# alibaba/pairec

Measured on AMD Instinct MI355X. Metric: ranked items/sec, 5k-cand DNN rank (recall top-5000 of 100M x 128 -> DNN3 -> fuse -> sort), higher is better.
Workload: dtype bf16x3; 1 GPU; configs[1]+[2]: recall 5k of 100000000x128 fp32 table in HBM -> 3-layer DNN rank (256-512-256-1, bf16 MFMA with split hi + lo operands = bf16x3, fp32-accurate scores) -> RankScore fusion (fp64) -> ItemRankScore sort; candidates_per_request=5000, table_rows=100000000, dim=128, table_dist=uniform, batches_in_flight=2, contexts=2, all_batches_on_predicted_thresholds=True, batches_re_run_after_a_failed_plan=0, parallelism=1 GPU

## Files before the change

### pairec_amd/csrc/recall.hip

```cpp
#include "common.hpp"
#include "bitonic_reg.hpp"
#include "split_sort.hpp"

#include <type_traits>

namespace pg {

typedef float f32x16 __attribute__((ext_vector_type(16)));
typedef float f32x4 __attribute__((ext_vector_type(4)));

constexpr int kPieceRows = 32;
constexpr int kPieceCols = 32;
constexpr int kPieceBytes = kPieceRows * kPieceCols * 4;
constexpr int kPieceDmas = kPieceBytes / 1024;
constexpr int kPieceQuads = kPieceCols / 4;
constexpr int kRingSlots = 4;
constexpr int kScanWaves = 8;
constexpr int kScanLdsRing = kScanWaves * kRingSlots * kPieceBytes;
constexpr int kStageCap = 280;
constexpr int kStageBytes = kStageCap * 12 + 512;
constexpr int kScanLds = kScanLdsRing + kScanWaves * kStageBytes;

__device__ __forceinline__ uint32_t f32_ordered_bits(float f) {
    const uint32_t b = __float_as_uint(f);
// ... 683 lines not shown
                for (int r = 0; r < 16; ++r) m = fmaxf(m, __fmaf_rn((float)acc[c][r], eu[c], -nxr[r]));
                cmask[c] = __builtin_amdgcn_ballot_w64(!(m < la[c]));
            } else if constexpr (I8) {
                int m = acc[c][0];
#pragma unroll
                for (int r = 1; r < 16; ++r) m = acc[c][r] > m ? acc[c][r] : m;
                cmask[c] = __builtin_amdgcn_ballot_w64(m >= cut[c]);
            } else {
                float m = acc[c][0];
#pragma unroll
                for (int r = 1; r < 16; ++r) m = fmaxf(m, acc[c][r]);
                cmask[c] = __builtin_amdgcn_ballot_w64(!(m < cut[c]));
            }
            any_mask |= cmask[c];
        }
        if (any_mask != 0) {
            const uint32_t row0 = cur_phys * kPieceRows;
#pragma unroll
            for (int c = 0; c < NQB; ++c) {
                if (cmask[c] == 0) continue;
                uint32_t m16 = 0;
#pragma unroll
                for (int r = 0; r < 16; ++r) {
                    if constexpr (L2 == 2) {
                        const float g = __fmaf_rn((float)acc[c][r], eu[c], -nxr[r]);
                        asm volatile("v_cmp_nlt_f32 vcc, %1, %2\n\tv_addc_co_u32 %0, vcc, %0, %0, vcc"
                                     : "+v"(m16) : "v"(g), "v"(la[c]) : "vcc");
                    } else if constexpr (I8)
                        asm volatile("v_cmp_ge_i32 vcc, %1, %2\n\tv_addc_co_u32 %0, vcc, %0, %0, vcc"
                                     : "+v"(m16) : "v"(acc[c][r]), "v"(cut[c]) : "vcc");
                    else
                        asm volatile("v_cmp_nlt_f32 vcc, %1, %2\n\tv_addc_co_u32 %0, vcc, %0, %0, vcc"
                                     : "+v"(m16) : "v"(acc[c][r]), "v"(cut[c]) : "vcc");
                }
                if (row0 + kPieceRows > a.row_end) {
#pragma unroll
                    for (int r = 0; r < 16; ++r)
                        if (row0 + (r & 3) + 8 * (r >> 2) + 4 * h >= a.row_end) m16 &= ~(1u << (15 - r));
                }
                for (;;) {
                    const bool p = m16 != 0;
                    const uint64_t bm = __builtin_amdgcn_ballot_w64(p);
                    if (bm == 0) break;
                    const uint32_t n = __popcll(bm);
                    if (st_n + n > (uint32_t)kCap) flush();
                    if (p) {
                        const int r = 15 - __builtin_ctz(m16);
                        const uint32_t pos = st_n + __builtin_amdgcn_mbcnt_hi((uint32_t)(bm >> 32),
                                                 __builtin_amdgcn_mbcnt_lo((uint32_t)bm, 0u));
                        st_row[pos] = row0 + (r & 3) + 8 * (r >> 2) + 4 * h;
                        st_q[pos] = (uint32_t)(c * 32 + i32);
                        m16 &= m16 - 1;
                    }
                    st_n += n;
                }
            }
        }
    }
    }
    if constexpr (QH == 1) flush();
    wait_vmcnt<0>();
}

__device__ __forceinline__ uint32_t rec_mask(const char* r, const float* __restrict__ thr_screen, uint32_t row_end, uint32_t& q,
                                             uint32_t& row0h) {
    typedef int i32x4 __attribute__((ext_vector_type(4)));
    const uint2 tag = *reinterpret_cast<const uint2*>(r + 64);
    q = tag.y & 255u;
    const uint32_t h = (tag.y >> 8) & 1u;
    row0h = tag.x + 4 * h;
    const int t = __float_as_int(thr_screen[q]);
    uint32_t m = 0;
#pragma unroll
    for (int jj = 0; jj < 4; ++jj) {
        const i32x4 v = *reinterpret_cast<const i32x4*>(r + 16 * jj);
#pragma unroll
        for (int e = 0; e < 4; ++e) {
            const int rr = 4 * jj + e;
            if (v[e] >= t && row0h + (rr & 3) + 8 * (rr >> 2) < row_end) m |= 1u << rr;
        }
    }
    return m;
}
constexpr uint32_t kRecPoolSlice = 8192;
__global__ __launch_bounds__(1024) void screen_decode_kernel(const char* __restrict__ rec, const uint32_t* __restrict__ rec_cnt,
                                                             uint32_t rec_cap, uint32_t rec_waves, const char* __restrict__ rec_pool,
                                                             uint32_t rec_pool_cap, const float* __restrict__ thr_screen, uint32_t row_end,
                                                             uint32_t* __restrict__ susp_cnt, uint32_t* __restrict__ susp,
                                                             uint32_t cap, uint32_t* __restrict__ overflow) {
    __shared__ uint32_t cntq[kMaxQueries], baseq[kMaxQueries], nreg[8];
    constexpr uint32_t kKeep = 12288;
    __shared__ uint2 keep[kKeep];
    const bool pool = blockIdx.x >= rec_waves / 8;
    if (threadIdx.x < kMaxQueries) cntq[threadIdx.x] = 0;
    if (threadIdx.x < 8) {
        uint32_t n;
        if (pool) {
            const uint32_t filled = rec_cnt[rec_waves] < rec_pool_cap ? rec_cnt[rec_waves] : rec_pool_cap;
            const uint32_t begin = (blockIdx.x - rec_waves / 8) * kRecPoolSlice;
            n = threadIdx.x == 0 && begin < filled ? (filled - begin < kRecPoolSlice ? filled - begin : kRecPoolSlice) : 0u;
        } else {
            const uint32_t n_raw = rec_cnt[blockIdx.x * 8 + threadIdx.x];
            n = n_raw < rec_cap ? n_raw : rec_cap;
        }
        nreg[threadIdx.x] = n;
    }
    __syncthreads();
    for (int pass = 0; pass < 2; ++pass) {
        uint32_t off = 0;
        for (uint32_t w = 0; w < 8; ++w) {
            const uint32_t n = nreg[w];
            const char* const base = pool ? rec_pool + (size_t)(blockIdx.x - rec_waves / 8) * kRecPoolSlice * kRecBytes
                                          : rec + (size_t)(blockIdx.x * 8 + w) * rec_cap * kRecBytes;
            for (uint32_t e = threadIdx.x; e < n; e += 1024) {
                uint32_t q, row0h, m;
                const uint32_t slot = off + e;
                if (pass == 1 && slot < kKeep) {
                    const uint2 kp = keep[slot];
                    row0h = kp.x;
                    q = kp.y & 0xffffu;
                    m = kp.y >> 16;
                } else {
                    m = rec_mask(base + (size_t)e * kRecBytes, thr_screen, row_end, q, row0h);
                    if (pass == 0 && slot < kKeep) keep[slot] = make_uint2(row0h, q | (m << 16));
                }
                if (m == 0) continue;
                const uint32_t nh = __popc(m);
                if (pass == 0) {
                    atomicAdd(&cntq[q], nh);
                } else {
                    uint32_t pos = baseq[q] + atomicAdd(&cntq[q], nh);
                    if (pos + nh > cap) { *overflow = 1u; continue; }
                    while (m) {
                        const uint32_t rr = __builtin_ctz(m);
                        m &= m - 1;
                        susp[(uint64_t)q * cap + pos++] = row0h + (rr & 3) + 8 * (rr >> 2);
                    }
                }
            }
            off += n;
        }
        __syncthreads();
        if (pass == 0 && threadIdx.x < kMaxQueries) {
            const uint32_t c = cntq[threadIdx.x];
            baseq[threadIdx.x] = c ? atomicAdd(&susp_cnt[threadIdx.x], c) : 0u;
            cntq[threadIdx.x] = 0;
        }
        __syncthreads();
    }
}

template <int DIM>
__device__ __forceinline__ void rescore_gather(f32x4 (&buf)[16], const float* __restrict__ tab, uint32_t row, int ph, int lane) {
#pragma unroll
    for (int i = 0; i < 16; ++i) {
        const uint32_t r_i = (uint32_t)__shfl((int)row, 4 * i + (lane >> 4), 64);
        buf[i] = reinterpret_cast<const f32x4*>(tab + (size_t)r_i * DIM + ph * 64)[lane & 15];
    }
}
template <int ROWB>
__device__ __forceinline__ void rescore_walk(const f32x4 (&buf)[16], char* my, const float* qs, int ph, int lane, float& s) {
#pragma unroll
    for (int i = 0; i < 16; ++i)
        *reinterpret_cast<f32x4*>(my + (4 * i + (lane >> 4)) * ROWB + (lane & 15) * 16) = buf[i];
    __builtin_amdgcn_fence(__ATOMIC_RELEASE, "wavefront");
    __builtin_amdgcn_wave_barrier();
#pragma unroll
    for (int k = 0; k < 16; ++k) {
        const float4 x = *reinterpret_cast<const float4*>(my + lane * ROWB + k * 16);
        const float4 y = *reinterpret_cast<const float4*>(&qs[ph * 64 + 4 * k]);
        s = __fmaf_rn(x.x, y.x, s);
        s = __fmaf_rn(x.y, y.y, s);
        s = __fmaf_rn(x.z, y.z, s);
        s = __fmaf_rn(x.w, y.w, s);
        if ((k & 3) == 3) __builtin_amdgcn_sched_barrier(0);
    }
    __builtin_amdgcn_wave_barrier();
}

template <int DIM, bool L2 = false>
__global__ __launch_bounds__(256) void rescore_kernel(const float* __restrict__ tab, const float* __restrict__ qpad,
                                                      const float* __restrict__ thr,
                                                      const uint32_t* __restrict__ susp,
                                                      const uint32_t* __restrict__ susp_cnt, uint32_t cap,
                                                      uint32_t* __restrict__ cnt, uint64_t* __restrict__ cand,
                                                      uint32_t* __restrict__ overflow, uint32_t scap, uint32_t n_rows,
                                                      const float* __restrict__ nx = nullptr, const float* __restrict__ nqv = nullptr,
                                                      RowFilter filter = RowFilter()) {
    constexpr int kRowB = 64 * 4 + 16;
    __shared__ __attribute__((aligned(16))) char tile[4][64 * kRowB];
    __shared__ __attribute__((aligned(16))) float qs[DIM];
    __shared__ uint32_t wsum[4];
    __shared__ uint32_t base_s;
    const uint32_t q = blockIdx.y;
    const uint32_t n_raw = susp_cnt[q];
    const uint32_t n = n_raw < scap ? n_raw : scap;
    if (blockIdx.x * 256u >= n) return;
    const int lane = threadIdx.x & 63, w = threadIdx.x >> 6;
    if (threadIdx.x < DIM) qs[threadIdx.x] = qpad[(size_t)q * DIM + threadIdx.x];
    const float thr_q = thr[q];
    __syncthreads();
    char* const my = tile[w];
    auto row_of = [&](uint32_t t0) -> uint32_t {
        const uint32_t e = t0 + threadIdx.x;
        const uint32_t r = e < n ? susp[(uint64_t)q * scap + e] : 0u;
        return r < n_rows ? r : 0u;
    };
    constexpr int NPH = DIM / 64;
    const uint32_t step = gridDim.x * 256u;
    uint32_t t0 = blockIdx.x * 256u;
    uint32_t row = row_of(t0);
    f32x4 va[16], vb[16];
    rescore_gather<DIM>(va, tab, row, 0, lane);
    for (; t0 < n; t0 += step) {
        const bool valid = t0 + threadIdx.x < n;
        const uint32_t row_next = t0 + step < n ? row_of(t0 + step) : 0u;
        float s = 0.0f;
        if constexpr (NPH == 1) {
            rescore_gather<DIM>(vb, tab, row_next, 0, lane);
            rescore_walk<kRowB>(va, my, qs, 0, lane, s);
        } else if constexpr (NPH == 2) {
            rescore_gather<DIM>(vb, tab, row, 1, lane);
            rescore_walk<kRowB>(va, my, qs, 0, lane, s);
            rescore_gather<DIM>(va, tab, row_next, 0, lane);
            rescore_walk<kRowB>(vb, my, qs, 1, lane, s);
        } else if constexpr (NPH == 3) {
            rescore_gather<DIM>(vb, tab, row, 1, lane);
            rescore_walk<kRowB>(va, my, qs, 0, lane, s);
            rescore_gather<DIM>(va, tab, row, 2, lane);
            rescore_walk<kRowB>(vb, my, qs, 1, lane, s);
            rescore_gather<DIM>(vb, tab, row_next, 0, lane);
            rescore_walk<kRowB>(va, my, qs, 2, lane, s);
        } else {
            static_assert(NPH == 4, "rescore_kernel: DIM 64, 128, 192 or 256");
            rescore_gather<DIM>(vb, tab, row, 1, lane);
            rescore_walk<kRowB>(va, my, qs, 0, lane, s);
            rescore_gather<DIM>(va, tab, row, 2, lane);
            rescore_walk<kRowB>(vb, my, qs, 1, lane, s);
            rescore_gather<DIM>(vb, tab, row, 3, lane);
            rescore_walk<kRowB>(va, my, qs, 2, lane, s);
            rescore_gather<DIM>(va, tab, row_next, 0, lane);
            rescore_walk<kRowB>(vb, my, qs, 3, lane, s);
        }
        if (NPH & 1) {
#pragma unroll
            for (int i = 0; i < 16; ++i) va[i] = vb[i];
        }
        if constexpr (L2) s = __fmaf_rn(2.0f, s, -(nx[row] + nqv[q]));
        const bool keep = valid && !(s < thr_q) && row_filter_pass(filter, row);
        const uint64_t m = __builtin_amdgcn_ballot_w64(keep);
        const uint32_t before = __builtin_amdgcn_mbcnt_hi((uint32_t)(m >> 32), __builtin_amdgcn_mbcnt_lo((uint32_t)m, 0u));
        if (lane == 0) wsum[w] = __popcll(m);
        __syncthreads();
        if (threadIdx.x == 0) {
            const uint32_t tot = wsum[0] + wsum[1] + wsum[2] + wsum[3];
            base_s = tot ? atomicAdd(&cnt[q], tot) : 0u;
        }
        __syncthreads();
        uint32_t pos = base_s + before;
        for (int j = 0; j < w; ++j) pos += wsum[j];
        if (keep) {
            if (pos < cap) cand[(uint64_t)q * cap + pos] = topk_key(s, row);
            else *overflow = 1u;
        }
        __syncthreads();
        row = row_next;
    }
    if (n_raw > scap && threadIdx.x == 0) *overflow = 1u;
}

__global__ void screen_prep_kernel(const float* __restrict__ qpad, uint32_t dim,
                                   uint4* __restrict__ qb16, float* __restrict__ eps) {
    const uint32_t KS = dim / 16;
    const uint32_t i = blockIdx.x * blockDim.x + threadIdx.x;
    if (i < (uint32_t)kScreenMaxNQB * KS * 64) {
        const uint32_t lane = i & 63, ks = (i >> 6) % KS, c = (i >> 6) / KS;
        const float* q = qpad + (size_t)(c * 32 + (lane & 31)) * dim + ks * 16 + 8 * (lane >> 5);
        uint32_t w[4];
        for (int e = 0; e < 4; ++e) {
            auto rne = [](float x) -> uint32_t {
                uint32_t b = __float_as_uint(x);
                if ((b & 0x7FFFFFFFu) > 0x7F800000u) return (b >> 16) | 0x40u;
                b += 0x7FFFu + ((b >> 16) & 1u);
                return b >> 16;
            };
            w[e] = rne(q[2 * e]) | (rne(q[2 * e + 1]) << 16);
        }
        qb16[i] = make_uint4(w[0], w[1], w[2], w[3]);
    }
    if (i < (uint32_t)kMaxQueries) {
        double ss = 0.0;
        for (uint32_t k = 0; k < dim; ++k) {
            const double v = (double)qpad[(size_t)i * dim + k];
            ss += v * v;
        }
        eps[i] = (float)(sqrt(ss) * (double)kScreenEps * 1.0001) + 1e-30f;
    }
}

__global__ void screen_thr_kernel(const float* __restrict__ thr, const float* __restrict__ eps, float max_norm,
                                  float* __restrict__ thr_screen) {
    const uint32_t q = threadIdx.x;
    if (q >= (uint32_t)kMaxQueries) return;
    const float t = thr[q], e = eps[q];
    float v = t;
    if (!(e == e) || e > 1e28f || !(t == t) || !(e * max_norm < 1e35f)) v = -__builtin_inff();
    thr_screen[q] = v;
}

__global__ __launch_bounds__(128) void screen_prep8_kernel(const float* __restrict__ qpad, uint32_t dim,
                                                            float max_norm, float resid, uint4* __restrict__ qb8,
                                                            float* __restrict__ eps, float* __restrict__ qscale) {
    __shared__ float sq[32];
    const uint32_t tid = threadIdx.x, c = blockIdx.x;
    {
        const uint32_t ql = tid >> 2, qi = c * 32 + ql, part = tid & 3, per = dim / 4;
        const float* q = qpad + (size_t)qi * dim + part * per;
        float mx = 0.0f;
        bool bad = false;
        for (uint32_t k = 0; k < per; ++k) {
            const float v = fabsf(q[k]);
            if (!(v <= 3.0e38f)) bad = true;
            mx = fmaxf(mx, v);
        }
        mx = fmaxf(mx, __shfl_xor(mx, 1, 64));
        mx = fmaxf(mx, __shfl_xor(mx, 2, 64));
        bad = (__shfl_xor((int)bad, 1, 64) | (int)bad) != 0;
        bad = (__shfl_xor((int)bad, 2, 64) | (int)bad) != 0;
        const float sc = fmaxf(mx / 127.0f, 1e-30f);
        double ss = 0.0, dd = 0.0;
        for (uint32_t k = 0; k < per; ++k) {
            const double v = (double)q[k];
            int Q = __float2int_rn(q[k] / sc);
            Q = Q > 127 ? 127 : (Q < -127 ? -127 : Q);
            const double d = v - (double)sc * (double)Q;
            ss += v * v;
            dd += d * d;
        }
        ss += __shfl_xor(ss, 1, 64);
        ss += __shfl_xor(ss, 2, 64);
        dd += __shfl_xor(dd, 1, 64);
        dd += __shfl_xor(dd, 2, 64);
        if (part == 0) {
            const double nq = sqrt(ss), dq = sqrt(dd);
            const double e = ((double)resid * nq + ((double)max_norm + (double)resid) * dq) * 1.0001 +
                             1e-5 * (double)max_norm * nq + 1e-30;
            eps[qi] = bad ? __builtin_nanf("") : (float)(e * 1.000001);
            qscale[qi] = sc;
            sq[ql] = sc;
        }
    }
    __syncthreads();
    const uint32_t KS = dim / 32;
    for (uint32_t i = tid; i < KS * 64; i += blockDim.x) {
        const uint32_t lane = i & 63, ks = i >> 6;
        const uint32_t ql = lane & 31;
        const float* q = qpad + (size_t)(c * 32 + ql) * dim + ks * 32 + 16 * (lane >> 5);
        const float sc = sq[ql];
        uint32_t w[4];
        for (int e = 0; e < 4; ++e) {
            uint32_t word = 0;
            for (int b = 0; b < 4; ++b) {
                int Q = __float2int_rn(q[4 * e + b] / sc);
                Q = Q > 127 ? 127 : (Q < -127 ? -127 : Q);
                word |= (uint32_t)(Q & 0xff) << (8 * b);
            }
            w[e] = word;
        }
        qb8[(c * KS + ks) * 64 + lane] = make_uint4(w[0], w[1], w[2], w[3]);
    }
}

__global__ void screen_thr8_kernel(const float* __restrict__ thr, const float* __restrict__ eps,
                                   const float* __restrict__ qscale, float s_x, float* __restrict__ thr_screen) {
    const uint32_t q = threadIdx.x;
    if (q >= (uint32_t)kMaxQueries) return;
    const float t = thr[q], e = eps[q];
    int T = (int)0x80000000;
    if (e == e && e <= 1e30f && t == t && t > -__builtin_inff()) {
        const double v = floor(((double)t - (double)e) / ((double)s_x * (double)qscale[q])) - 1.0;
        T = v >= 2147483647.0 ? 0x7fffffff : (v <= -2147483648.0 ? (int)0x80000000 : (int)v);
    }
    thr_screen[q] = __int_as_float(T);
}

__global__ void screen_thr8_l2_kernel(const float* __restrict__ thr, const float* __restrict__ eps, const float* __restrict__ qscale,
                                      const float* __restrict__ nqv, float s_x, float max_norm, float* __restrict__ a_out,
                                      float* __restrict__ b_out, int per_row) {
    const uint32_t q = threadIdx.x;
    if (q >= (uint32_t)kMaxQueries) return;
    const float t = thr[q], e = eps[q];
    const double nq = (double)nqv[q], N = (double)max_norm;
    const double sq = (double)s_x * (double)qscale[q];
    float A = -__builtin_inff(), B = 0.0f;
    if (e == e && e <= 1e30f && t == t && t > -__builtin_inff() && sq > 0.0 && nq == nq && nq < 1e30) {
        const double delta = 2e-6 * (N * N + nq + 2.0 * N * sqrt(nq)) + 1e-30;
        if (per_row) {
            const double c = (double)t - 2.0 * delta + nq - 2.0 * (double)e;
            A = (float)(c - fabs(c) * 1e-6 - 1e-30);
            B = (float)(2.0 * sq);
            if (!(A == A) || !(B == B) || B > 1e30f) { A = -__builtin_inff(); B = 0.0f; }
        } else {
            const double a = (((double)t - delta + nq) * 0.5 - (double)e) / sq;
            const double b = 0.5 / sq;
            A = (float)(a - fabs(a) * 1e-6 - 1.0);
            B = (float)(b * (1.0 - 1e-6));
            if (!(A == A) || !(B == B) || B > 1e30f) { A = -__builtin_inff(); B = 0.0f; }
        }
    }
    a_out[q] = A;
    b_out[q] = B;
}
__global__ void block_nxmin_kernel(const float* __restrict__ nx, uint64_t rows, float* __restrict__ out, uint32_t nblocks,
                                   double* __restrict__ stats) {
    const uint32_t b = blockIdx.x * blockDim.x + threadIdx.x;
    double slack = 0.0, sum = 0.0;
    if (b < nblocks) {
        float m = __builtin_inff();
        for (uint32_t i = 0; i < (uint32_t)kPieceRows; ++i) {
            const uint64_t r = (uint64_t)b * kPieceRows + i;
            if (r < rows) m = fminf(m, nx[r]);
// ... 1233 lines not shown
    }
    j->stage2 = false;
    if (screen && !j->l2 && t->dim == 128 && t->shadow_is_i8 && !j->screen4m && !j->screen4 && !kn.no_r2 &&
        (double)t->wide_susp > kn.r2_min_factor * (double)j->k) {
        if ((rc = ensure_table_r2(ctx, t))) return rc;
        j->stage2 = t->r2_ok;
    }
    j->predict = j->pred_observe = false;
    if (screen && !j->l2 && !j->filter.col && t->dim == 128 && t->shadow_is_i8 && j->plans[0] == kPilot && !j->skip_pilot && !kn.no_predict &&
        rows >= kn.predict_min_rows && j->k < rows / 64) {
        if ((rc = ensure_pred_model(ctx, t))) return rc;
        pg_table* tm = const_cast<pg_table*>(t);
        std::lock_guard<std::mutex> build_guard(g_stats_build_mu);
        if (t->pred_model) {
            if (tm->pred_k != j->k) {
                PG_HIP(hipMemsetAsync(t->d_pred + 128 + 128 * 128, 0, 24, ctx->stream));
                tm->pred_k = j->k;
                tm->pred_n = tm->pred_sum = tm->pred_sum2 = 0.0;
                tm->pred_backoff = 4;
            }
            j->pred_observe = !(j->nq <= (uint32_t)kI4MaxQueries && t->pred_n >= 8192.0);
            if (tm->pred_backoff > 0) {
                --tm->pred_backoff;
            } else if (t->pred_n >= 1024.0) {
                const double mean = t->pred_sum / t->pred_n;
                const double var = t->pred_sum2 / t->pred_n - mean * mean;
                const double sd = var > 0.0 ? sqrt(var) : 0.0;
                if (mean > 0.5 && sd <= 0.025 * mean) {
                    j->predict = true;
                    j->z_lo = mean - kn.predict_sigmas * sd - 0.002 * mean;
                    for (int i = j->n_plans; i > 0; --i) j->plans[i] = j->plans[i - 1];
                    j->plans[0] = kPredict;
                    j->n_plans++;
                }
            }
        }
    }
    return index_plan_prepare(j);
}

namespace {
struct PlanRun {
    RecallJob* j;
    pg_ctx* ctx;
    const pg_table* t;
    RecallScratch& rs;
    uint32_t n_ev = 0;
    int cur = 0;
    bool susp2_clean = false;
    bool susp_clean = true;
    bool no_i8 = false;
    bool last_full_screened = false;
    bool last_was_i4m = false;
    bool last_was_r2 = false;
    bool exact_chunks = false;

    explicit PlanRun(RecallJob* job) : j(job), ctx(job->ctx), t(job->t), rs(job->rs) {}

    int scan_range(uint32_t rb, uint32_t cb, uint32_t st, bool thr_is_open, bool allow_i4 = false) {
        std::vector<hipEvent_t>& pool = *j->events;
        while (pool.size() < 2 * (size_t)(n_ev + 1)) {
            hipEvent_t e;
            PG_HIP(hipEventCreate(&e));
            pool.push_back(e);
        }
        if (j->timers) PG_HIP(hipEventRecord(pool[2 * n_ev], ctx->stream));
        const uint32_t nq = j->nq;
        if (j->screen && !thr_is_open && !exact_chunks) {
            ScreenArgs sa;
            sa.tab16 = t->shadow_is_i8 ? (const void*)t->d8 : (const void*)t->d16;
            sa.blk_norm2 = t->dnorm2;
            sa.eps_unit = rs.eps;
            sa.qb16 = rs.qb16;
            sa.thr_screen = rs.thr_screen;
            sa.susp_cnt = rs.susp_cnt;
            sa.susp = rs.susp;
            sa.overflow = rs.overflow;
            sa.cap = rs.cap;
            sa.nq = nq;
            sa.rb_begin = rb;
            sa.rb_end = rb + cb;
            sa.row_end = j->rows;
            sa.stride = st;
            sa.perm_mul = j->perm_mul;
            sa.perm_mod = j->sample_blocks;
            int rc2;
            const bool records = t->shadow_is_i8 && nq > 128;
            sa.rec = nullptr;
            sa.rec_cnt = nullptr;
            sa.rec_cap = 0;
            sa.rec_pool = nullptr;
            sa.rec_pool_cap = sa.rec_waves = 0;
            sa.early_share = records ? ctx->knobs.screen_early_share : ctx->knobs.screen_early_share_narrow;
            sa.blk_nxmin = j->l2 && !j->l2_per_row ? t->d_nxmin : nullptr;
            sa.nx_rows = j->l2 && j->l2_per_row ? t->d_nx : nullptr;
            sa.l2_b = j->l2 ? rs.thr_ref : nullptr;
            const uint32_t rec_waves = (uint32_t)ctx->num_cus * 8u;
            if (records) {
                const uint64_t rsc = t->rec_scale ? t->rec_scale : 1;
                uint32_t cap_w = (uint32_t)(((uint64_t)kMaxQueries * j->k * 4 * rsc / rec_waves + 255) / 256 * 256);
                const uint32_t pairs = (uint32_t)ctx->num_cus * 4u;
                const uint32_t pb = (kCandSlack / 2 / kPieceRows + pairs - 1) / pairs;
                const uint32_t es = sa.early_share > 512 ? sa.early_share : 1024 - sa.early_share;
                uint32_t eb = (uint32_t)(((uint64_t)pb * es + 512) >> 10) + 1;
                if (eb > pb) eb = pb;
                const uint32_t floor_w = eb * 512;
                if (cap_w < floor_w) cap_w = floor_w;
                const uint32_t pool_cap = (uint32_t)(((uint64_t)kMaxQueries * j->k * 2 * rsc + kRecPoolSlice - 1) / kRecPoolSlice * kRecPoolSlice);
                const size_t head = ((size_t)(rec_waves + 1) * 4 + 255) & ~(size_t)255;
                void* p;
                if ((rc2 = scratch_reserve(ctx, 11, head + ((size_t)rec_waves * cap_w + pool_cap) * kRecBytes, &p))) return rc2;
                sa.rec_cnt = (uint32_t*)p;
                sa.rec = (char*)p + head;
                sa.rec_cap = cap_w;
                sa.rec_pool = sa.rec + (size_t)rec_waves * cap_w * kRecBytes;
                sa.rec_pool_cap = pool_cap;
                sa.rec_waves = rec_waves;
                PG_HIP(hipMemsetAsync(sa.rec_cnt, 0, (size_t)(rec_waves + 1) * 4, ctx->stream));
            }
            if (!susp_clean) PG_HIP(hipMemsetAsync(rs.susp_cnt, 0, sizeof(uint32_t) * kMaxQueries, ctx->stream));
            susp_clean = false;
            last_full_screened = true;
            last_was_r2 = false;
            const bool i4 = j->screen4 && allow_i4 && st == 1 && (rb & 1) == 0 && (((rb + cb) & 1) == 0 || rb + cb == j->nblocks);
            const bool i4m = j->screen4m && allow_i4 && st == 1 && (rb & 1) == 0 && (((rb + cb) & 1) == 0 || rb + cb == j->nblocks);
            const uint32_t scap = i4 ? rs.cap * (uint32_t)(kMaxQueries / kI4MaxQueries) : rs.cap;
            const uint64_t r_begin = (uint64_t)rb * kPieceRows;
            const uint64_t r_end = (uint64_t)(rb + cb) * kPieceRows < j->rows ? (uint64_t)(rb + cb) * kPieceRows : j->rows;
            if (i4) {
                if ((rc2 = screen4_launch(ctx, t, rs, nq, (uint32_t)r_begin, (uint32_t)r_end, scap, j->l2 ? rs.pred_ms : nullptr))) return rc2;
                j->scan_bytes += (r_end - r_begin) * (j->l2 ? 72 : 68);
            } else if (i4m) {
                if ((rc2 = screen4m_launch(ctx, t, rs, nq, (uint32_t)r_begin, (uint32_t)r_end, rs.cap * (uint32_t)(kMaxQueries / kI4mMaxQueries), susp2_clean))) return rc2;
                susp2_clean = false;
                j->scan_bytes += (r_end - r_begin) * 68;
                last_was_i4m = true;
            } else {
                last_was_i4m = false;
                if ((rc2 = dispatch_screen(ctx, t->dim, t->shadow_is_i8, sa))) return rc2;
                if (records) {
                    screen_decode_kernel<<<rec_waves / 8 + sa.rec_pool_cap / kRecPoolSlice, 1024, 0, ctx->stream>>>(
                        sa.rec, sa.rec_cnt, sa.rec_cap, rec_waves, sa.rec_pool, sa.rec_pool_cap, rs.thr_screen, j->rows,
                                                                            rs.susp_cnt, rs.susp, rs.cap, rs.overflow);
                    PG_HIP(hipGetLastError());
                }
                j->scan_bytes += (uint64_t)cb * kPieceRows * t->dim * (t->shadow_is_i8 ? 1 : 2);
            }
            j->scanned_rows += (uint64_t)cb * kPieceRows;
            const dim3 rg(i4 ? screen4_rescore_blocks() : kRescoreBlocksPerQuery, nq);
            const bool r2 = j->stage2 && t->shadow_is_i8 && !i4 && !i4m && !j->l2 && t->dim == 128;
            if (r2) {
                if ((rc2 = rescreen16_launch(ctx, t, rs, nq))) return rc2;
                last_was_r2 = true;
                rescore_kernel<128><<<rg, 256, 0, ctx->stream>>>(t->d, rs.qpad, rs.thr, rs.susp2, rs.susp2w_cnt, rs.cap,
                                                                 rs.cnt, rs.cand[cur], rs.overflow, rs.cap, j->rows, nullptr, nullptr, j->filter);
            } else if (j->l2)
                rescore_kernel<128, true><<<rg, 256, 0, ctx->stream>>>(t->d, rs.qpad, rs.thr, rs.susp, rs.susp_cnt, rs.cap, rs.cnt,
                                                                       rs.cand[cur], rs.overflow, scap, j->rows, t->d_nx, rs.pred_ms, j->filter);
            else if (t->dim == 64)
                rescore_kernel<64><<<rg, 256, 0, ctx->stream>>>(t->d, rs.qpad, rs.thr, rs.susp, rs.susp_cnt, rs.cap,
                                                                rs.cnt, rs.cand[cur], rs.overflow, scap, j->rows, nullptr, nullptr, j->filter);
            else if (i4m)
                rescore_kernel<128><<<rg, 256, 0, ctx->stream>>>(t->d, rs.qpad, rs.thr, rs.susp2, rs.susp2_cnt, rs.cap,
                                                                 rs.cnt, rs.cand[cur], rs.overflow, rs.cap, j->rows, nullptr, nullptr, j->filter);
            else
                rescore_kernel<128><<<rg, 256, 0, ctx->stream>>>(t->d, rs.qpad, rs.thr, rs.susp, rs.susp_cnt, rs.cap,
                                                                 rs.cnt, rs.cand[cur], rs.overflow, scap, j->rows, nullptr, nullptr, j->filter);
            PG_HIP(hipGetLastError());
        } else {
            last_full_screened = false;
            ScanArgs a;
            a.tab = t->d;
            a.qpad = rs.qpad;
            a.thr = rs.thr;
            a.cnt = rs.cnt;
            a.cand = rs.cand[cur];
            a.overflow = rs.overflow;
            a.cap = rs.cap;
            a.nq = nq;
            a.group_q = nq > (uint32_t)kMaxQueriesExact ? (uint32_t)kMaxQueriesExact : 0u;
            a.nq_launch = a.group_q ? a.group_q : nq;
            a.rb_begin = rb;
            a.rb_end = rb + cb;
            a.row_end = j->rows;
            a.stride = st;
            a.perm_mul = j->perm_mul;
            a.perm_mod = j->sample_blocks;
            a.nx = j->l2 ? t->d_nx : nullptr;
            a.nqv = j->l2 ? rs.pred_ms : nullptr;
            a.filter = j->filter;
            int rc2;
            if ((rc2 = dispatch_scan(ctx, t->dim, a))) return rc2;
            j->scan_bytes += (uint64_t)cb * kPieceRows * t->dim * 4;
            j->scanned_rows += (uint64_t)cb * kPieceRows;
        }
        if (j->timers) PG_HIP(hipEventRecord(pool[2 * n_ev + 1], ctx->stream));
        ++n_ev;
        return PG_OK;
    }
    int refresh(uint32_t kk, bool last = false) {
        int rc2;
        if ((rc2 = launch_select(ctx, j->nq, rs.cand[cur], rs.cand[cur ^ 1], rs.cnt, rs.thr, rs.cap, kk, 0, rs.cnt_seen))) return rc2;
        if (j->screen && !no_i8 && !(last && !j->l2)) {
            if (j->l2) screen_thr8_l2_kernel<<<1, kMaxQueries, 0, ctx->stream>>>(rs.thr, rs.eps, rs.qscale, rs.pred_ms, t->s8, t->max_norm,
                                                                                rs.thr_screen, rs.thr_ref, j->l2_per_row ? 1 : 0);
            else if (t->shadow_is_i8) screen_thr8_kernel<<<1, kMaxQueries, 0, ctx->stream>>>(rs.thr, rs.eps, rs.qscale, t->s8, rs.thr_screen);
            else screen_thr_kernel<<<1, kMaxQueries, 0, ctx->stream>>>(rs.thr, rs.eps, t->max_norm, rs.thr_screen);
            PG_HIP(hipGetLastError());
        }
        cur ^= 1;
        return PG_OK;
    }
    int refine(uint32_t kk) {
        int rc2;
        if ((rc2 = launch_select(ctx, j->nq, rs.cand[cur], rs.cand[cur ^ 1], rs.cnt, rs.thr, rs.cap, kk, 1))) return rc2;
        if (j->screen) {
            if (t->shadow_is_i8) screen_thr8_kernel<<<1, kMaxQueries, 0, ctx->stream>>>(rs.thr, rs.eps, rs.qscale, t->s8, rs.thr_screen);
            else screen_thr_kernel<<<1, kMaxQueries, 0, ctx->stream>>>(rs.thr, rs.eps, t->max_norm, rs.thr_screen);
            PG_HIP(hipGetLastError());
        }
        return PG_OK;
    }
    int grow_scan(uint32_t nb, uint32_t st, uint32_t kk, double growth, bool safe) {
        uint32_t rb = 0;
        while (rb < nb) {
            uint32_t chunk_rows;
            if (rb == 0) {
                chunk_rows = next_pow2(8 * kk);
                if (chunk_rows < 2048) chunk_rows = 2048;
                if (chunk_rows > kFirstChunkRows || chunk_rows < kk) chunk_rows = kFirstChunkRows;
            } else {
                const uint64_t grow = (uint64_t)((double)rb * kPieceRows * (growth - 1.0));
                chunk_rows = grow > 0xFFFFFFE0ull ? 0xFFFFFFE0u : (uint32_t)grow;
            }
            if (safe && chunk_rows > kCandSlack / 2) chunk_rows = kCandSlack / 2;
            uint32_t cb = chunk_rows / kPieceRows;
            if (cb > nb - rb) cb = nb - rb;
            int rc2;
            if ((rc2 = scan_range(rb, cb, st, rb == 0))) return rc2;
            rb += cb;
            if ((rc2 = refresh(kk))) return rc2;
        }
        return PG_OK;
    }
};
}

int recall_job_enqueue(RecallJob* j) {
    pg_ctx* ctx = j->ctx;
    const pg_table* t = j->t;
    const Knobs& kn = ctx->knobs;
    if (j->next_plan >= j->n_plans) {
        set_error("recall: candidate overflow in safe mode (internal error)");
        return PG_ERR_DEVICE;
    }
    const int plan = j->plans[j->next_plan];
    int rc;
    if ((rc = recall_scratch(ctx, t->dim, j->k, &j->rs))) return rc;
    j->d_count = j->rs.overflow + 1;
    if (plan == kIndexPlan) return index_plan_enqueue(j, kStatusCopyWords);
    PlanRun r(j);
    RecallScratch& rs = j->rs;
    recall_init_kernel<<<(kMaxQueries * t->dim + 255) / 256, 256, 0, ctx->stream>>>(
        j->d_queries, j->nq, t->dim, rs.qpad, rs.thr, rs.cnt, rs.overflow);
    PG_HIP(hipGetLastError());
    if (j->l2) {
        query_norm2_kernel<<<1, kMaxQueries, 0, ctx->stream>>>(rs.qpad, t->dim, rs.pred_ms);
        PG_HIP(hipGetLastError());
    }
    r.no_i8 = plan == kPredict && j->screen4;
    if (j->screen) {
        if (!r.no_i8) {
            if (t->shadow_is_i8)
                screen_prep8_kernel<<<j->nq <= 32 ? 1u : (j->nq <= 64 ? 2u : (j->nq <= 128 ? 4u : 8u)), 128, 0, ctx->stream>>>(
                    rs.qpad, t->dim, t->max_norm, t->resid8, rs.qb16, rs.eps, rs.qscale);
            else
                screen_prep_kernel<<<(kScreenMaxNQB * (t->dim / 16) * 64 + 255) / 256, 256, 0, ctx->stream>>>(
                    rs.qpad, t->dim, rs.qb16, rs.eps);
            PG_HIP(hipGetLastError());
        }
        if (j->screen4 && (rc = screen4_prep_launch(ctx, t, rs))) return rc;
        if (j->screen4m) {
            if ((rc = screen4m_prep_launch(ctx, rs, j->nq))) return rc;
            r.susp2_clean = true;
        }
        if (j->stage2 && (rc = rescreen16_prep_launch(ctx, t, rs, j->nq))) return rc;
    }
    const bool observe = j->pred_observe && (plan == kPilot || plan == kPredict);
    if (observe || plan == kPredict) {
        pred_query_kernel<<<j->nq, 128, 0, ctx->stream>>>(rs.qpad, t->d_pred, rs.pred_ms, plan == kPredict ? rs.thr : nullptr,
                                                          (float)j->z_lo);
        PG_HIP(hipGetLastError());
    }
    while (j->events->size() < 2) {
        hipEvent_t e;
        PG_HIP(hipEventCreate(&e));
        j->events->push_back(e);
    }
    bool refined = false;
    r.n_ev = 1;
    j->timers = !ctx->timers_off;
    if (j->timers) PG_HIP(hipEventRecord((*j->events)[0], ctx->stream));
    if (plan == kPredict && !r.no_i8) {
        screen_thr8_kernel<<<1, kMaxQueries, 0, ctx->stream>>>(rs.thr, rs.eps, rs.qscale, t->s8, rs.thr_screen);
        PG_HIP(hipGetLastError());
    }
    if (plan == kPilot || plan == kPredict) {
      if (plan == kPilot) {
        const uint32_t seed_rows = kn.seed_rows;
        const uint64_t sample_rows = (uint64_t)j->sample_blocks * kPieceRows;
        if (j->screen && kn.pilot_growth <= 0.0 && sample_rows > 8ull * seed_rows && j->k_pilot < seed_rows / 4) {
            const double mu = (double)seed_rows * (double)j->k_pilot / (double)sample_rows;
            uint32_t m0 = 1;
            for (double term = exp(-mu), cdf = term; 1.0 - cdf > 1e-9 && m0 < seed_rows; ++m0) {
                term *= mu / (double)m0;
                cdf += term;
            }
            ++m0;
            const uint32_t sb = seed_rows / kPieceRows;
            if ((rc = r.scan_range(0, sb, j->stride, true))) return rc;
// ... 782 lines not shown
```

Before: 276.8 million ranked items/s.

## Rework rescore kernel: per-wave staged output, deeper row prefetch, filter specialization

The rescore kernel's per-iteration block-wide compaction is replaced. It used three __syncthreads and one atomic per block per iteration. Each wave now stages kept keys in LDS and flushes them with a single wave-level atomic when the stage fills. Suspect row indices are prefetched two iterations ahead, shuffles in the gather are split from the loads with a sched barrier, and occupancy is hinted at 2 blocks per CU. A new FILT template parameter drops the row-filter check when no filter is set. The trade-offs are more LDS per block, more atomics in flight across waves, and reordered candidate output.

Measured after the change: 278.2 million ranked items/s, median of 2. Within noise of the previous version (+0.5%).

```diff
diff --git a/pairec_amd/csrc/recall.hip b/pairec_amd/csrc/recall.hip
--- a/pairec_amd/csrc/recall.hip
+++ b/pairec_amd/csrc/recall.hip
@@ -859,11 +859,12 @@
 
 template <int DIM>
 __device__ __forceinline__ void rescore_gather(f32x4 (&buf)[16], const float* __restrict__ tab, uint32_t row, int ph, int lane) {
-#pragma unroll
-    for (int i = 0; i < 16; ++i) {
-        const uint32_t r_i = (uint32_t)__shfl((int)row, 4 * i + (lane >> 4), 64);
-        buf[i] = reinterpret_cast<const f32x4*>(tab + (size_t)r_i * DIM + ph * 64)[lane & 15];
-    }
+    uint32_t r[16];
+#pragma unroll
+    for (int i = 0; i < 16; ++i) r[i] = (uint32_t)__shfl((int)row, 4 * i + (lane >> 4), 64);
+    __builtin_amdgcn_sched_barrier(0);
+#pragma unroll
+    for (int i = 0; i < 16; ++i) buf[i] = reinterpret_cast<const f32x4*>(tab + (size_t)r[i] * DIM + ph * 64)[lane & 15];
 }
 template <int ROWB>
 __device__ __forceinline__ void rescore_walk(const f32x4 (&buf)[16], char* my, const float* qs, int ph, int lane, float& s) {
@@ -885,8 +886,8 @@
     __builtin_amdgcn_wave_barrier();
 }
 
-template <int DIM, bool L2 = false>
-__global__ __launch_bounds__(256) void rescore_kernel(const float* __restrict__ tab, const float* __restrict__ qpad,
+template <int DIM, bool L2 = false, bool FILT = false>
+__global__ __launch_bounds__(256, DIM <= 128 ? 2 : 1) void rescore_kernel(const float* __restrict__ tab, const float* __restrict__ qpad,
                                                       const float* __restrict__ thr,
                                                       const uint32_t* __restrict__ susp,
                                                       const uint32_t* __restrict__ susp_cnt, uint32_t cap,
@@ -897,8 +898,8 @@
     constexpr int kRowB = 64 * 4 + 16;
     __shared__ __attribute__((aligned(16))) char tile[4][64 * kRowB];
     __shared__ __attribute__((aligned(16))) float qs[DIM];
-    __shared__ uint32_t wsum[4];
-    __shared__ uint32_t base_s;
+    constexpr uint32_t kStageChunks = 4;
+    __shared__ uint64_t stage[4][kStageChunks * 64];
     const uint32_t q = blockIdx.y;
     const uint32_t n_raw = susp_cnt[q];
     const uint32_t n = n_raw < scap ? n_raw : scap;
@@ -908,27 +909,47 @@
     const float thr_q = thr[q];
     __syncthreads();
     char* const my = tile[w];
-    auto row_of = [&](uint32_t t0) -> uint32_t {
+    auto row_raw = [&](uint32_t t0) -> uint32_t {
         const uint32_t e = t0 + threadIdx.x;
-        const uint32_t r = e < n ? susp[(uint64_t)q * scap + e] : 0u;
-        return r < n_rows ? r : 0u;
+        return susp[(uint64_t)q * scap + (e < n ? e : n - 1u)];
+    };
+    auto row_of = [&](uint32_t t0, uint32_t r) -> uint32_t { return ((t0 + threadIdx.x < n) & (r < n_rows)) ? r : 0u; };
+    uint32_t staged = 0;
+    auto flush = [&]() {
+        uint32_t base = 0;
+        if (lane == 0) base = atomicAdd(&cnt[q], staged);
+        base = (uint32_t)__builtin_amdgcn_readfirstlane((int)base);
+        __builtin_amdgcn_fence(__ATOMIC_RELEASE, "wavefront");
+        __builtin_amdgcn_wave_barrier();
+        for (uint32_t e = lane; e < staged; e += 64) {
+            if (base + e < cap) cand[(uint64_t)q * cap + base + e] = stage[w][e];
+            else *overflow = 1u;
+        }
+        __builtin_amdgcn_wave_barrier();
+        staged = 0;
     };
     constexpr int NPH = DIM / 64;
     const uint32_t step = gridDim.x * 256u;
     uint32_t t0 = blockIdx.x * 256u;
-    uint32_t row = row_of(t0);
+    uint32_t row = row_raw(t0), row_next = row_raw(t0 + step);
+    row = row_of(t0, row);
+    row_next = row_of(t0 + step, row_next);
     f32x4 va[16], vb[16];
     rescore_gather<DIM>(va, tab, row, 0, lane);
     for (; t0 < n; t0 += step) {
         const bool valid = t0 + threadIdx.x < n;
-        const uint32_t row_next = t0 + step < n ? row_of(t0 + step) : 0u;
+        float nxr = 0.0f;
+        if constexpr (L2) nxr = nx[row];
+        uint32_t row_nn;
         float s = 0.0f;
         if constexpr (NPH == 1) {
+            row_nn = row_raw(t0 + 2 * step);
             rescore_gather<DIM>(vb, tab, row_next, 0, lane);
             rescore_walk<kRowB>(va, my, qs, 0, lane, s);
         } else if constexpr (NPH == 2) {
             rescore_gather<DIM>(vb, tab, row, 1, lane);
             rescore_walk<kRowB>(va, my, qs, 0, lane, s);
+            row_nn = row_raw(t0 + 2 * step);
             rescore_gather<DIM>(va, tab, row_next, 0, lane);
             rescore_walk<kRowB>(vb, my, qs, 1, lane, s);
         } else if constexpr (NPH == 3) {
@@ -936,6 +957,7 @@
             rescore_walk<kRowB>(va, my, qs, 0, lane, s);
             rescore_gather<DIM>(va, tab, row, 2, lane);
             rescore_walk<kRowB>(vb, my, qs, 1, lane, s);
+            row_nn = row_raw(t0 + 2 * step);
             rescore_gather<DIM>(vb, tab, row_next, 0, lane);
             rescore_walk<kRowB>(va, my, qs, 2, lane, s);
         } else {
@@ -946,6 +968,7 @@
             rescore_walk<kRowB>(vb, my, qs, 1, lane, s);
             rescore_gather<DIM>(vb, tab, row, 3, lane);
             rescore_walk<kRowB>(va, my, qs, 2, lane, s);
+            row_nn = row_raw(t0 + 2 * step);
             rescore_gather<DIM>(va, tab, row_next, 0, lane);
             rescore_walk<kRowB>(vb, my, qs, 3, lane, s);
         }
@@ -953,27 +976,29 @@
 #pragma unroll
             for (int i = 0; i < 16; ++i) va[i] = vb[i];
         }
-        if constexpr (L2) s = __fmaf_rn(2.0f, s, -(nx[row] + nqv[q]));
-        const bool keep = valid && !(s < thr_q) && row_filter_pass(filter, row);
+        if constexpr (L2) s = __fmaf_rn(2.0f, s, -(nxr + nqv[q]));
+        bool keep = valid && !(s < thr_q);
+        if constexpr (FILT) keep = keep && row_filter_pass(filter, row);
         const uint64_t m = __builtin_amdgcn_ballot_w64(keep);
         const uint32_t before = __builtin_amdgcn_mbcnt_hi((uint32_t)(m >> 32), __builtin_amdgcn_mbcnt_lo((uint32_t)m, 0u));
-        if (lane == 0) wsum[w] = __popcll(m);
-        __syncthreads();
-        if (threadIdx.x == 0) {
-            const uint32_t tot = wsum[0] + wsum[1] + wsum[2] + wsum[3];
-            base_s = tot ? atomicAdd(&cnt[q], tot) : 0u;
-        }
-        __syncthreads();
-        uint32_t pos = base_s + before;
-        for (int j = 0; j < w; ++j) pos += wsum[j];
-        if (keep) {
-            if (pos < cap) cand[(uint64_t)q * cap + pos] = topk_key(s, row);
-            else *overflow = 1u;
-        }
-        __syncthreads();
+        if (keep) stage[w][staged + before] = topk_key(s, row);
+        staged += (uint32_t)__popcll(m);
+        if (staged > (kStageChunks - 1) * 64u) flush();
         row = row_next;
-    }
+        row_next = row_of(t0 + 2 * step, row_nn);
+    }
+    if (staged) flush();
     if (n_raw > scap && threadIdx.x == 0) *overflow = 1u;
+}
+
+template <int DIM, bool L2>
+static void rescore_launch(dim3 grid, hipStream_t stream, const float* tab, const float* qpad, const float* thr, const uint32_t* susp,
+                           const uint32_t* susp_cnt, uint32_t cap, uint32_t* cnt, uint64_t* cand, uint32_t* overflow, uint32_t scap,
+                           uint32_t n_rows, const float* nx, const float* nqv, const RowFilter& filter) {
+    if (filter.col)
+        rescore_kernel<DIM, L2, true><<<grid, 256, 0, stream>>>(tab, qpad, thr, susp, susp_cnt, cap, cnt, cand, overflow, scap, n_rows, nx, nqv, filter);
+    else
+        rescore_kernel<DIM, L2><<<grid, 256, 0, stream>>>(tab, qpad, thr, susp, susp_cnt, cap, cnt, cand, overflow, scap, n_rows, nx, nqv);
 }
 
 __global__ void screen_prep_kernel(const float* __restrict__ qpad, uint32_t dim,
@@ -2513,20 +2538,20 @@
             if (r2) {
                 if ((rc2 = rescreen16_launch(ctx, t, rs, nq))) return rc2;
                 last_was_r2 = true;
-                rescore_kernel<128><<<rg, 256, 0, ctx->stream>>>(t->d, rs.qpad, rs.thr, rs.susp2, rs.susp2w_cnt, rs.cap,
-                                                                 rs.cnt, rs.cand[cur], rs.overflow, rs.cap, j->rows, nullptr, nullptr, j->filter);
+                rescore_launch<128, false>(rg, ctx->stream, t->d, rs.qpad, rs.thr, rs.susp2, rs.susp2w_cnt, rs.cap,
+                                           rs.cnt, rs.cand[cur], rs.overflow, rs.cap, j->rows, nullptr, nullptr, j->filter);
             } else if (j->l2)
-                rescore_kernel<128, true><<<rg, 256, 0, ctx->stream>>>(t->d, rs.qpad, rs.thr, rs.susp, rs.susp_cnt, rs.cap, rs.cnt,
-                                                                       rs.cand[cur], rs.overflow, scap, j->rows, t->d_nx, rs.pred_ms, j->filter);
+                rescore_launch<128, true>(rg, ctx->stream, t->d, rs.qpad, rs.thr, rs.susp, rs.susp_cnt, rs.cap, rs.cnt,
+                                          rs.cand[cur], rs.overflow, scap, j->rows, t->d_nx, rs.pred_ms, j->filter);
             else if (t->dim == 64)
-                rescore_kernel<64><<<rg, 256, 0, ctx->stream>>>(t->d, rs.qpad, rs.thr, rs.susp, rs.susp_cnt, rs.cap,
-                                                                rs.cnt, rs.cand[cur], rs.overflow, scap, j->rows, nullptr, nullptr, j->filter);
+                rescore_launch<64, false>(rg, ctx->stream, t->d, rs.qpad, rs.thr, rs.susp, rs.susp_cnt, rs.cap,
+                                          rs.cnt, rs.cand[cur], rs.overflow, scap, j->rows, nullptr, nullptr, j->filter);
             else if (i4m)
-                rescore_kernel<128><<<rg, 256, 0, ctx->stream>>>(t->d, rs.qpad, rs.thr, rs.susp2, rs.susp2_cnt, rs.cap,
-                                                                 rs.cnt, rs.cand[cur], rs.overflow, rs.cap, j->rows, nullptr, nullptr, j->filter);
+                rescore_launch<128, false>(rg, ctx->stream, t->d, rs.qpad, rs.thr, rs.susp2, rs.susp2_cnt, rs.cap,
+                                           rs.cnt, rs.cand[cur], rs.overflow, rs.cap, j->rows, nullptr, nullptr, j->filter);
             else
-                rescore_kernel<128><<<rg, 256, 0, ctx->stream>>>(t->d, rs.qpad, rs.thr, rs.susp, rs.susp_cnt, rs.cap,
-                                                                 rs.cnt, rs.cand[cur], rs.overflow, scap, j->rows, nullptr, nullptr, j->filter);
+                rescore_launch<128, false>(rg, ctx->stream, t->d, rs.qpad, rs.thr, rs.susp, rs.susp_cnt, rs.cap,
+                                           rs.cnt, rs.cand[cur], rs.overflow, scap, j->rows, nullptr, nullptr, j->filter);
             PG_HIP(hipGetLastError());
         } else {
             last_full_screened = false;
```
